# Martinsos/edlib

Hardware: AMD Instinct MI355X
Metric: GCUPS (cell updates/s), 1M x 150bp HW reads vs 5Mb target (higher is better)
Workload: dtype u32

## Files before the change

edlib_amd/csrc/engine.hpp:

```cpp
#pragma once
#include "../../include/edlib_amd.h"
#include "common.hpp"
#include "pair_kernels.hpp"
#include "lanepair.hpp"
#include "reads_kernels.hpp"
#include "cross_kernels.hpp"
#include "window_kernels.hpp"
#include "strands.hpp"

#include <chrono>
#include <deque>
#include <functional>
#include <memory>
#include <vector>

namespace edlib_amd {

struct Tables {
    uint8_t tlut[256];
    uint8_t idToByte[256];
    int sigmaT = 0;
    uint32_t presence[8];
    uint16_t eqtbl[256];
    std::vector<uint8_t> eq8;
// ... 147 lines not shown
    Event evRun0_, evRun1_, evA_, evB_;

    DevBuf<uint8_t> d_in_;
    PinBuf h_in_;
    DevBuf<uint8_t> d_qpool_, d_tpool_, d_tlut_, d_idToByte_, d_eq8_;
    DevBuf<uint16_t> d_eqtbl_;
    hipError_t uploadEq8();
    DevBuf<uint32_t> d_presence_;
    DevBuf<long long> d_qoff_, d_toff_;

    std::vector<int> emptyUnits_, readUnits_, pairUnits_;
    std::vector<int> longUnits_;
    std::vector<int> pairNow_;
    int beginRun(hipError_t guardStatus);
    int enqueueWordSteps();
    int endRun();
    void resetRecords(std::vector<UnitResult>& res);
    void answerEmptyUnits(std::vector<UnitResult>& res);
    int runFlatPhase(std::vector<UnitResult>& res, Lap& lap);
    int runLongReads(std::vector<UnitResult>& res, Lap& lap);
    int runPairPhase(std::vector<UnitResult>& res, Lap& lap);
    int runStartsPhase(std::vector<UnitResult>& res, Lap& lap);
    int runPathsPhase(std::vector<UnitResult>& res, Lap& lap);
    void startStats();
    bool flatDone_ = false;

    struct ReadGroup {
        int nwords = 0, nslots = 0, numSegments = 1, segLen = 0, warm = 0, mMin = 0, mMax = 0;
        std::vector<int> perm;
        DevBuf<int> d_perm, d_qlen, d_kinit, d_alphaExtra, d_segBest, d_segCnt, d_segPos;
        DevBuf<int> d_best, d_total, d_pos, d_flags;
        DevBuf<uint32_t> d_peq;
        bool zeroCopy = false; PinBuf hostOut;
        std::vector<int> ovfSlots; std::vector<long long> ovfOff; DevBuf<int> d_ovfPool;
        DevBuf<int> d_lvMap, d_lvBest, d_lvCnt, d_lvPos; std::vector<int> lvMap; int lvS = 0, lvCap = 0; bool lvValid = false;
        DevBuf<int> d_list;
        int nreal = -1;
        bool mates = false; DevBuf<int> d_win;
    };
    static constexpr int kLastLevelCap = 16;
    int listOpenSlots(ReadGroup& g, int kDone, std::vector<int>& out);
    DevBuf<uint8_t> d_selTmp_;
    std::vector<std::unique_ptr<ReadGroup>> groups_;
    DevBuf<uint32_t> d_tpk_, d_trows_;
    DevBuf<unsigned long long> d_wordSteps_;
    PinBuf h_wordSteps_; bool wordStepsPending_ = false;
    DevBuf<unsigned long long> d_ringSteps_; PinBuf h_ringSteps_; bool ringStepsUsed_ = false;
    unsigned long long* ringStepsCounter();
    bool banded_ = false;
    int syms_ = 4;
    int packTarget();
    int runReads();
    int makeGroup(const std::vector<int>& units, int words, std::unique_ptr<ReadGroup>& g, long long oneRoundWaves = 0);
    int runGroupScans(ReadGroup& g, bool fullOnly);
    int runGroupExact(ReadGroup& g);
    int collectGroup(ReadGroup& g, std::vector<UnitResult>& res);
    int seedThreshold(const ReadGroup& g, bool fullOnly) const;
    int buildSeedIndex();
    int runSeedPass(ReadGroup& g, int k);
    DevBuf<uint32_t> d_seedCnt_, d_seedOff_, d_seedPos_;
    DevBuf<uint8_t> d_seedTmp_;
    bool hits_ = false, hitsHaveRun_ = false;
    HitListBuffers hitList_;
    HitRows hostHits_;
    DevBuf<int> d_hitSlotUnit_;
    DevBuf<long long> d_hitTotal_;
    int runReadHits();
    int scanGroupHits(ReadGroup& g, int slotBase);
    int hitsScanBanded(ReadGroup& g, int slotBase, const int* d_slotmap, int nlanes, int numSegments, int segLen, int warm);
    struct Piece { long long off; int len; int thr; };
    int scanPieces(const std::vector<Piece>& pieces, bool filter, std::vector<std::pair<int, int>>* cand,
                   std::vector<uint8_t>* overflow, std::vector<int>* best);
    int solveLongReads(std::vector<UnitResult>& res, std::vector<int>& fallback);
    bool filterScan_ = false;
    struct ChainArgs { const uint32_t* in = nullptr; uint32_t* out = nullptr; const int* src = nullptr; int inLanes = 0, blocks = 0; const int* rowBase = nullptr; };
    ChainArgs chain_;
    int solveTallFull(const std::vector<int>& units, std::vector<UnitResult>& res, std::vector<int>& handBack);
    int collectReads(std::vector<UnitResult>& res);
    bool readsCollected_ = true;
    int scanGroup(ReadGroup& g, int mode, const int* d_slotmap, int nlanes, int kcap, const int* d_kinit,
                  int numSegments, int segLen, int warm, int* segBest, int* segCnt, int* segPos, int cap,
                  const long long* posOff, const int* posCap, bool unbanded = false,
                  unsigned long long* wordSteps = nullptr, const uint32_t* peqDense = nullptr,
                  const int* qlenDense = nullptr, int peqBottom = 0);

    DevBuf<PairDesc> d_descs_;
    DevBuf<unsigned long long> d_peq64_;
    DevBuf<StoreEntry> d_store_;
    DevBuf<int> d_aux_, d_out3_, d_outScore_, d_outCount_, d_outLast_, d_posPool_, d_opsLen_, d_alpha_;
    DevBuf<uint8_t> d_ops_;
    DevBuf<long long> d_opsOff_;
    int solve(int mode, bool wantPositions, bool wantPath, const std::vector<UnitSpec>& units, SolveOut& out,
              int ring = 0, int ringH = 1);
    int solveChunk(int mode, bool wantPositions, bool wantPath, const std::vector<UnitSpec>& units,
                   size_t a, size_t b, SolveOut& out, int ring, int ringH);
    static const int kWide = -1;
    static const int kRing32 = -2;
    bool ring32_fits(const std::vector<UnitSpec>& units, size_t a, size_t b, int G) const;
    DevBuf<unsigned long long> d_wide_; DevBuf<unsigned> d_wabort_; PinBuf h_wabort_;
    int wideCap_ = -1;
    struct WidePlan { int slots = 1; size_t perLaunch = 1; };
    int planWide(int mode, PairDesc* descs, size_t n, WidePlan& plan);
    int launchWide(int mode, const PairScanArgs& a, const PairDesc* hostDescs, size_t n, const WidePlan& plan);
    int checkWide();
    bool wideSerial_ = false;
    bool wideGateHeld_ = false;
    void wideGateRelease();
    int solveWideSplit(const std::vector<UnitSpec>& units, std::vector<int>& out, int ring = 0);
    struct KnownSplit { long long qoff; int m; long long toff; int T; int score; int row, left, right; };
    std::vector<KnownSplit> knownSplits_;
    int solveGlobalDistances(const std::vector<UnitSpec>& units, std::vector<int>& score, std::vector<OpsOut>* paths = nullptr);
    int solveSemiGlobal(int mode, bool wantPositions, const std::vector<UnitSpec>& units, SolveOut& out);
    int solveSemiGlobalUnits(int mode, bool wantPositions, const std::vector<UnitSpec>& units, SolveOut& out);
    int solveBanded(const BandLadder& ladder, bool wantPositions, const std::vector<UnitSpec>& units, SolveOut& out);
    int alphabetLengthsBegin(hipEvent_t after = nullptr);
    bool alphaDeferred_ = false;
    int alphabetLengthsEnd(std::vector<UnitResult>& res);
    std::vector<int> alphaUnits_; bool alphaOnHost_ = false, alphaPending_ = false; long long alphaBytes_ = 0;
    hipStream_t side_ = nullptr;
    DevBuf<int> d_alphaIdx_, d_alphaOut_; PinBuf alphaPin_;
    struct PathPiece { long long qoff; int m; long long toff; int T; int score; };
    int hirschbergLevel(const std::vector<PathPiece>& big, std::vector<int>& splitRow,
                        std::vector<int>& leftScore, std::vector<int>& rightScore);
    int solvePaths(const std::vector<PathPiece>& jobs, std::vector<OpsOut>& opsOut, std::vector<int>& status);
    std::vector<std::shared_ptr<PinBuf>> opsKeep_;
    std::deque<std::vector<uint8_t>> opsOwned_;

    int qlen(int u) const { return (int)(qoff_[u + 1] - qoff_[u]); }
    long long tbase(int u) const { return shared_ ? toff_[0] : toff_[u]; }
    int tlen(int u) const { return shared_ ? (int)(toff_[1] - toff_[0]) : (int)(toff_[u + 1] - toff_[u]); }

    void scanTimerStart();
    void scanTimerStop();
    std::vector<std::pair<hipEvent_t, hipEvent_t>> scanEvents_;
    size_t scanEventsUsed_ = 0;

    std::vector<UnitResult> results_, work_;
    std::vector<UnitSpec> startUnits_; std::vector<std::pair<int, int>> startWhere_; std::vector<int> live_;
    bool haveResults_ = false;
    long long algoBase_ = -1;
    bool algoDirty_ = false;
    std::vector<int> pairSpecsFor_;
    std::vector<UnitSpec> pairSpecs_, selScratch_; std::vector<size_t> whoScratch_; std::vector<int> lvlScratch_, scoreMain_;
    SolveOut soMain_, soLevel_;
    int pairSpecsVersion_ = 0, levelSpecsVersion_ = -1, shapeVersion_ = -1, alphaIsPairsVersion_ = -1;
    bool alphaIsPairs_ = false;
    struct PairShape { size_t minBlocks = 0, maxBlocks = 0; int minLenLo = 0, minLenHi = 0, maxDiff = 0; } shape_;
    long long levelPeqWords_ = 0;
    bool levelAllReady_ = false;
    PinBuf h_levelSpecs_, h_levelScore_;
    DevBuf<LevelSpec> d_levelSpecs_;
    DevBuf<PairDesc> d_descsAll_;
    DevBuf<unsigned long long> d_peqAll_;
    hipStream_t aux_ = nullptr;
    Event evLevelIn_, evLevelPeq_;
    int prepareLevelAll(const std::vector<UnitSpec>& units);
    std::function<void()> whileScanning_;
    int runLevelAll(const std::vector<UnitSpec>& units, int ring, int ringH, int ringBlocks, int cap, int kcap, int nbMax);
    int laneSpecsVersion_ = -1;
    long long lanePlaneWords_ = -1, laneTgtWords_ = 0;
    bool laneReady_ = false;
    PinBuf h_laneUnits_, h_laneScore_;
    DevBuf<lanepair::LaneUnit> d_laneUnits_;
    DevBuf<lanepair::Plane2> d_lanePlanes_;
    DevBuf<lanepair::Tgt2> d_laneTgts_;
    DevBuf<int> d_laneFlags_, d_laneScore_;
    Event evLanePack_;
// ... 89 lines not shown
```

edlib_amd/csrc/engine_reads.hip:

```cpp
#include "engine.hpp"

#include <algorithm>
#include <chrono>
#include <cmath>
#include <condition_variable>
#include <cstring>
#include <mutex>
#include <thread>

namespace edlib_amd {

__global__ void __launch_bounds__(256)
seed_thresholds_kernel(int* __restrict__ kinit, const int* __restrict__ best, const int* __restrict__ cnt, int n)
{
    const int i = blockIdx.x * blockDim.x + threadIdx.x;
    if (i < n && cnt[i] > 0 && best[i] < kinit[i]) kinit[i] = best[i];
}


int Batch::scanGroup(ReadGroup& g, int mode, const int* d_slotmap, int nlanes, int kcap, const int* d_kinit,
                     int numSegments, int segLen, int warm, int* segBest, int* segCnt, int* segPos, int cap,
                     const long long* posOff, const int* posCap, bool unbanded, unsigned long long* wordSteps,
                     const uint32_t* peqDense, const int* qlenDense, int peqBottom)
{
    ReadScanArgs a{};
    a.peq = peqDense ? peqDense : g.d_peq.p; a.tpk = d_tpk_.p; a.trows = d_trows_.p; a.targetLength = tlen(0);
    if (mode == EDLIB_MODE_SHW) a.targetLength = (int)std::min<long long>(a.targetLength, 64LL * g.nwords + 1);
    a.qlen = qlenDense ? qlenDense : g.d_qlen.p; a.kinit = d_kinit; a.slotmap = d_slotmap; a.nlanes = nlanes;
    a.numSegments = numSegments; a.segLen = segLen; a.warm = warm;
    a.segBest = segBest; a.segCnt = segCnt; a.segPos = segPos; a.cap = cap;
    a.posOff = posOff; a.posCap = posCap;
    a.kcap = kcap; a.wordSteps = wordSteps ? wordSteps : d_wordSteps_.p;
    a.filter = filterScan_ ? 1 : 0;
    a.bottomAligned = peqBottom;
    a.chainIn = chain_.in; a.chainOut = chain_.out; a.chainSrc = chain_.src; a.chainInLanes = chain_.inLanes;
    a.chainBlocks = chain_.blocks; a.rowBase = chain_.rowBase;
    const bool chained = chain_.in != nullptr || chain_.out != nullptr;
    static const bool dbg = getenv("EDLIB_AMD_DEBUG") != nullptr;
    if (dbg) {
        EDLIB_AMD_HIP(hipStreamSynchronize(stream_));
        fprintf(stderr, "[edlib_amd] scanGroup nwords=%d mode=%d nlanes=%d S=%d segLen=%d warm=%d cap=%d kcap=%d slotmap=%p posOff=%p rows=%s\n",
                g.nwords, mode, nlanes, numSegments, segLen, warm, cap, kcap, (const void*)d_slotmap, (const void*)posOff,
                peqBottom > 1 ? "delay" : (peqBottom ? "bottom" : "top"));
    }
    scanTimerStart();
    const bool longGroup = g.nwords > kMaxReadWords;
    const long long colsScanned = std::min<long long>(a.targetLength, (long long)numSegments * segLen) + (long long)(numSegments - 1) * warm;
    const bool fullHeight = banded_ && mode == EDLIB_MODE_HW && unbanded && (chained || syms_ > 4 || longGroup);
    const bool bandedKernel = !fullHeight && banded_ && mode == EDLIB_MODE_HW && (!unbanded || syms_ > 4 || longGroup);
    if (peqBottom && (fullHeight || bandedKernel)) EDLIB_AMD_HIP(hipErrorInvalidValue);
    if (fullHeight) {
        EDLIB_AMD_HIP(launch_scan_reads_full(g.nwords, syms_, a, stream_));
        stats.word_steps += (long long)((nlanes + 63) / 64 * 64) * g.nwords * colsScanned;
    } else if (bandedKernel) EDLIB_AMD_HIP(launch_scan_reads_banded(g.nwords, syms_, a, stream_));
    else {
        EDLIB_AMD_HIP(launch_scan_reads(g.nwords, mode, a, stream_));
        stats.word_steps += (long long)((nlanes + 63) / 64 * 64) * g.nwords * colsScanned;
    }
    scanTimerStop();
    if (dbg) {
        EDLIB_AMD_HIP(hipStreamSynchronize(stream_));
        fprintf(stderr, "[edlib_amd] scanGroup done\n");
    }
    return 0;
}

void plan_segments(int nlanes, int T, int mode, int warmFull, long long wantWaves,
                          int& S, int& segLen, int& warm, int minSegCols)
{
    S = 1; segLen = roundup(T, 16); warm = 0;
    if (mode != EDLIB_MODE_HW) return;
    const long long nrblk = ((long long)nlanes + 63) / 64;
    long long want = (wantWaves + nrblk - 1) / nrblk;
    want = std::max(1LL, std::min<long long>(want, std::min(65535, std::max(1, T / minSegCols))));
    if (warmFull > 0) want = std::max(1LL, std::min<long long>(want, std::max<long long>(1, T / (4LL * warmFull))));
    segLen = roundup((int)((T + want - 1) / want), 16);
    S = (T + segLen - 1) / segLen;
    warm = warmFull;
}

int Batch::runReads()
{
    if (groups_.empty()) return 0;
    stats.path |= 1;
    bool seed = false;
    for (auto& gp : groups_) seed = seed || seedThreshold(*gp, false) >= 0;
    if (seed && buildSeedIndex()) return 1;
    for (auto& gp : groups_) if (runGroupScans(*gp, false)) return 1;
    const int mode = (cfg_.mode == EDLIB_MODE_HW || cfg_.mode == EDLIB_MODE_SHW) ? (int)cfg_.mode : (int)EDLIB_MODE_NW;
    for (auto& gp : groups_)
        if (gp->mates) EDLIB_AMD_HIP(launch_resolve_strands(gp->d_perm.p, gp->d_best.p, gp->d_total.p, gp->nslots, mode, cfg_.k,
                                                            gp->d_win.p, stream_));
    for (auto& gp : groups_) if (runGroupExact(*gp)) return 1;
    return 0;
}

int Batch::runGroupScans(ReadGroup& g, bool fullOnly)
{
    const int T = tlen(0);
    const int mode = (cfg_.mode == EDLIB_MODE_HW || cfg_.mode == EDLIB_MODE_SHW) ? (int)cfg_.mode : (int)EDLIB_MODE_NW;
    const bool banded = banded_ && mode == EDLIB_MODE_HW;
    const int kNoCap = 0x3fffffff;
    static const bool dbgLadder = getenv("EDLIB_AMD_DEBUG") != nullptr;
    EDLIB_AMD_HIP(launch_build_peq_reads(g.nwords, syms_, d_qpool_.p, d_qoff_.p, g.d_perm.p, g.nslots,
                                         d_eqtbl_.p, d_presence_.p, cfg_.k, g.d_peq.p, g.d_qlen.p,
                                         g.d_kinit.p, g.d_alphaExtra.p, stream_));
    const int kSeed = seedThreshold(g, fullOnly);
    const int kFirstMax = kSeed >= 0 ? kSeed : std::max(8, g.nwords / 2);
    int kFirst = (kSeed >= 0 && cfg_.k >= 0) ? std::min(kSeed, cfg_.k) : kFirstMax;
    bool twoPass = !fullOnly && banded && (cfg_.k < 0 || cfg_.k > kFirst) && 32 * g.nwords > kFirst;
    std::vector<int> ladder;
    g.lvValid = false;
    auto probe_scan = [&](const std::vector<int>& map, int kc, std::vector<int>& bestOut) -> int {
        const int nm = (int)map.size();
        int S2, segLen2, warm2;
        plan_segments(nm, T, mode, g.warm, 16384, S2, segLen2, warm2);
// ... 77 lines not shown
        if (runSeedPass(g, kFirst)) return 1;
        if (twoPass) {
            if (listOpenSlots(g, kFirst, todo)) return 1;
            haveTodo = true;
            if (g.nreal < 0) { g.nreal = 0; for (int u : g.perm) g.nreal += u >= 0; }
            if (g.nslots >= 16384 && todo.size() * 10 > (size_t)g.nreal && todo.size() >= 32) {
                const size_t nsm = std::min<size_t>(2048, todo.size());
                std::vector<int> sample(nsm);
                for (size_t i = 0; i < nsm; ++i) sample[i] = todo[i * todo.size() / nsm];
                if (price_ladder(sample, todo.size(), g.nreal)) return 1;
            }
        }
    } else {
        if (scanGroup(g, mode, nullptr, g.nslots, twoPass ? kFirst : kNoCap, g.d_kinit.p, g.numSegments, g.segLen,
                      g.warm, g.d_segBest.p, g.d_segCnt.p, g.d_segPos.p, 8, nullptr, nullptr, fullOnly)) return 1;
        const bool chained = chain_.in != nullptr || chain_.out != nullptr;
        EDLIB_AMD_HIP(launch_merge_segments(g.d_segBest.p, g.d_segCnt.p, g.d_segPos.p, g.numSegments, 8,
                                            g.nslots, nullptr, 16, g.d_best.p, g.d_total.p, g.d_pos.p,
                                            g.d_flags.p, stream_, chained ? kOvfRescan : kOvfGatherGroup));
    }
    ladder.push_back(kNoCap);
    int kDone = kFirst;
    for (size_t lv = 0; twoPass && lv < ladder.size(); ++lv) {
        const int kcapL = ladder[lv];
        const bool last = kcapL == kNoCap;
        if (!haveTodo && listOpenSlots(g, kDone, todo)) return 1;
        haveTodo = false;
        if (todo.empty()) break;
        {
            const size_t no = todo.size();
            int S2, segLen2, warm2;
            plan_segments((int)no, T, mode, g.warm, 65536, S2, segLen2, warm2);
            const size_t items = no * (size_t)S2;
            const int capL = last ? kLastLevelCap : 8;
            EDLIB_AMD_HIP(g.d_lvMap.ensure(no)); EDLIB_AMD_HIP(g.d_lvBest.ensure(items)); EDLIB_AMD_HIP(g.d_lvCnt.ensure(items));
            EDLIB_AMD_HIP(g.d_lvPos.ensure(items * capL));
            int *d_map = g.d_lvMap.p, *d_sb = g.d_lvBest.p, *d_sc = g.d_lvCnt.p, *d_sp = g.d_lvPos.p;
            EDLIB_AMD_HIP(hipMemcpyAsync(d_map, todo.data(), no * sizeof(int), hipMemcpyHostToDevice, stream_));
            bool plain = false;
            if (last && no >= 4096) {
                const int np2 = 64;
                std::vector<int> sub(np2);
                for (int i = 0; i < np2; ++i) sub[i] = todo[(size_t)((long long)i * no / np2)];
                int S3, segLen3, warm3;
                plan_segments(np2, T, mode, g.warm, 16384, S3, segLen3, warm3);
                const size_t it3 = (size_t)np2 * S3;
                DevBuf<int> d_m3, d_b3, d_c3, d_p3; DevBuf<unsigned long long> d_ws;
                EDLIB_AMD_HIP(d_m3.alloc(np2)); EDLIB_AMD_HIP(d_b3.alloc(it3)); EDLIB_AMD_HIP(d_c3.alloc(it3));
                EDLIB_AMD_HIP(d_p3.alloc(it3 * 8)); EDLIB_AMD_HIP(d_ws.alloc(1));
                EDLIB_AMD_HIP(hipMemcpyAsync(d_m3.p, sub.data(), np2 * sizeof(int), hipMemcpyHostToDevice, stream_));
                EDLIB_AMD_HIP(hipMemsetAsync(d_ws.p, 0, sizeof(unsigned long long), stream_));
                if (scanGroup(g, mode, d_m3.p, np2, kNoCap, g.d_kinit.p, S3, segLen3, warm3,
                              d_b3.p, d_c3.p, d_p3.p, 8, nullptr, nullptr, false, d_ws.p)) return 1;
                unsigned long long ws = 0;
                EDLIB_AMD_HIP(hipMemcpyAsync(&ws, d_ws.p, sizeof ws, hipMemcpyDeviceToHost, stream_));
                EDLIB_AMD_HIP(hipStreamSynchronize(stream_));
                const double cols = (double)np2 * ((double)T + (double)(S3 - 1) * warm3);
                plain = (double)ws >= 0.85 * g.nwords * cols;
                stats.word_steps += (long long)ws;
            }
            const bool bottomOk = plain && mode == EDLIB_MODE_HW && syms_ == 4 && g.nwords <= kMaxReadWords &&
                                  chain_.in == nullptr && chain_.out == nullptr;
            const int bottom = !bottomOk ? 0 : (delay_rows_fit(g.nwords, g.mMax) ? 1 + kDelayRows : 1);
            const size_t no64 = (no + 63) / 64 * 64;
            std::vector<int> perm2(no64, -1);
            for (size_t i = 0; i < no; ++i) perm2[i] = g.perm[todo[i]];
            DevBuf<int> d_perm2, d_qlen2, d_kinit2, d_extra2; DevBuf<uint32_t> d_peq2;
            EDLIB_AMD_HIP(d_perm2.alloc(no64)); EDLIB_AMD_HIP(d_qlen2.alloc(no64)); EDLIB_AMD_HIP(d_kinit2.alloc(no64));
            EDLIB_AMD_HIP(d_extra2.alloc(no64)); EDLIB_AMD_HIP(d_peq2.alloc(no64 * (size_t)syms_ * g.nwords));
            EDLIB_AMD_HIP(hipMemcpyAsync(d_perm2.p, perm2.data(), no64 * sizeof(int), hipMemcpyHostToDevice, stream_));
            EDLIB_AMD_HIP(launch_build_peq_reads(g.nwords, syms_, d_qpool_.p, d_qoff_.p, d_perm2.p, (int)no64,
                                                 d_eqtbl_.p, d_presence_.p, cfg_.k, d_peq2.p, d_qlen2.p,
                                                 d_kinit2.p, d_extra2.p, stream_, bottom));
            const int seedCols = 4096;
            DevBuf<int> d_b0, d_c0, d_p0;
            if (mode == EDLIB_MODE_HW && last && no >= 4096 && S2 > 1 && T >= 16 * seedCols) {
                EDLIB_AMD_HIP(d_b0.alloc(no)); EDLIB_AMD_HIP(d_c0.alloc(no)); EDLIB_AMD_HIP(d_p0.alloc(no * 8));
                if (scanGroup(g, mode, nullptr, (int)no, kcapL, d_kinit2.p, 1, seedCols, 0,
                              d_b0.p, d_c0.p, d_p0.p, 8, nullptr, nullptr, plain, nullptr, d_peq2.p, d_qlen2.p, bottom)) return 1;
                hipLaunchKernelGGL(seed_thresholds_kernel, dim3((unsigned)((no + 255) / 256)), dim3(256), 0, stream_,
                                   d_kinit2.p, d_b0.p, d_c0.p, (int)no);
                EDLIB_AMD_HIP(hipGetLastError());
            }
            if (scanGroup(g, mode, nullptr, (int)no, kcapL, d_kinit2.p, S2, segLen2, warm2,
                          d_sb, d_sc, d_sp, capL, nullptr, nullptr, plain, nullptr, d_peq2.p, d_qlen2.p, bottom)) return 1;
            EDLIB_AMD_HIP(launch_merge_segments(d_sb, d_sc, d_sp, S2, capL, (int)no, d_map, 16,
                                                g.d_best.p, g.d_total.p, g.d_pos.p, g.d_flags.p, stream_,
                                                last ? kOvfGatherLevel : kOvfRescan));
            EDLIB_AMD_HIP(hipStreamSynchronize(stream_));
            if (last) { g.lvValid = true; g.lvS = S2; g.lvCap = capL; g.lvMap.swap(todo); }
            if (dbgLadder) fprintf(stderr, "[edlib_amd] level kcap=%d: %zu slots rescanned (plain=%d)\n", kcapL, no, (int)plain);
        }
        kDone = kcapL;
    }
    return 0;
}

int Batch::listOpenSlots(ReadGroup& g, int kDone, std::vector<int>& out)
{
    size_t tmp = 0;
    EDLIB_AMD_HIP(select_slots_scratch_bytes(g.nslots, &tmp));
    EDLIB_AMD_HIP(d_selTmp_.ensure(tmp));
    EDLIB_AMD_HIP(g.d_list.ensure((size_t)g.nslots + 1));
    int* count = g.d_list.p + g.nslots;
    EDLIB_AMD_HIP(launch_select_open_slots(g.d_perm.p, g.d_total.p, g.d_qlen.p, cfg_.k, kDone, g.nslots, g.d_list.p, count,
                                           d_selTmp_.p, d_selTmp_.bytes(), stream_, g.mates));
    int n = 0;
    EDLIB_AMD_HIP(hipMemcpyAsync(&n, count, sizeof(int), hipMemcpyDeviceToHost, stream_));
    EDLIB_AMD_HIP(hipStreamSynchronize(stream_));
    out.resize((size_t)n);
    if (n > 0) {
        EDLIB_AMD_HIP(hipMemcpyAsync(out.data(), g.d_list.p, (size_t)n * sizeof(int), hipMemcpyDeviceToHost, stream_));
        EDLIB_AMD_HIP(hipStreamSynchronize(stream_));
    }
    return 0;
}


int Batch::seedThreshold(const ReadGroup& g, bool fullOnly) const
{
    const long long T = tlen(0);
    if (fullOnly || !banded_ || cfg_.mode != EDLIB_MODE_HW || syms_ != 4 || cfg_.additionalEqualitiesLength > 0 ||
        g.nwords > kMaxReadWords || chain_.in != nullptr || chain_.out != nullptr)
        return -1;
    if (T < 64LL * 32 * g.nwords || g.nslots < 1024 || (long long)g.nslots * T < (1LL << 30)) return -1;
    int kf = -1;
    for (int k = 16; k >= 0 && kf < 0; --k) {
        const int L = g.mMin / (k + 1);
        if (L >= kSeedQ && (double)(k + 1) * (double)T <= std::ldexp(1.0, 2 * L) / 8.0) kf = k;
    }
    return (kf >= 0 && kf >= std::min(8, cfg_.k >= 0 ? cfg_.k : 8)) ? kf : -1;
}

int Batch::buildSeedIndex()
{
    const int T = tlen(0);
    EDLIB_AMD_HIP(d_seedCnt_.ensure((size_t)kSeedBuckets + 1));
    EDLIB_AMD_HIP(d_seedOff_.ensure((size_t)kSeedBuckets + 1));
    EDLIB_AMD_HIP(d_seedPos_.ensure((size_t)T));
    size_t tmp = 0;
    EDLIB_AMD_HIP(seed_index_scratch_bytes(&tmp));
    EDLIB_AMD_HIP(d_seedTmp_.ensure(tmp));
    scanTimerStart();
    EDLIB_AMD_HIP(launch_build_seed_index(d_tpk_.p, T, d_seedCnt_.p, d_seedOff_.p, d_seedPos_.p, d_seedTmp_.p,
                                          d_seedTmp_.bytes(), stream_));
    scanTimerStop();
    return 0;
}

int Batch::runSeedPass(ReadGroup& g, int k)
{
    const int T = tlen(0);
    DevBuf<int> d_back;
    EDLIB_AMD_HIP(d_back.alloc((size_t)g.nslots + 1));
    int* backCount = d_back.p + g.nslots;
    EDLIB_AMD_HIP(hipMemsetAsync(backCount, 0, sizeof(int), stream_));
    SeedArgs a{};
    a.peq = g.d_peq.p; a.qlen = g.d_qlen.p; a.perm = g.d_perm.p; a.tpk = d_tpk_.p; a.targetLength = T;
    a.seedOff = d_seedOff_.p; a.seedPos = d_seedPos_.p; a.nslots = g.nslots; a.k = k;
    a.best = g.d_best.p; a.total = g.d_total.p; a.pos = g.d_pos.p; a.flags = g.d_flags.p;
    a.backSlots = d_back.p; a.backCount = backCount; a.wordSteps = d_wordSteps_.p;
    scanTimerStart();
    EDLIB_AMD_HIP(launch_seed_verify(g.nwords, a, stream_));
    scanTimerStop();
    int nb = 0;
    EDLIB_AMD_HIP(hipMemcpyAsync(&nb, backCount, sizeof(int), hipMemcpyDeviceToHost, stream_));
    EDLIB_AMD_HIP(hipStreamSynchronize(stream_));
    static const bool dbg = getenv("EDLIB_AMD_DEBUG") != nullptr;
// ... 320 lines not shown
```

edlib_amd/csrc/reads_kernels.hip:

```cpp
#include "reads_kernels.hpp"
#include "reads_scan.hpp"
#include "reads_column_asm.hpp"

namespace edlib_amd {


__global__ void __launch_bounds__(256)
pack_target_2bit_kernel(const uint8_t* __restrict__ raw, const uint8_t* __restrict__ lut,
                        int T, u32* __restrict__ tpk, int nwords)
{
    __shared__ uint8_t s_lut[256];
    s_lut[threadIdx.x] = lut[threadIdx.x];
    __syncthreads();
    const int w = blockIdx.x * blockDim.x + threadIdx.x;
    if (w >= nwords) return;
    const int base = w * 16;
    u32 out = 0;
    if (base + 16 <= T) {
        const uint4 v = *reinterpret_cast<const uint4*>(raw + base);
        const u32 d[4] = {v.x, v.y, v.z, v.w};
#pragma unroll
        for (int i = 0; i < 16; ++i)
            out |= (u32)(s_lut[(d[i >> 2] >> ((i & 3) * 8)) & 0xFF] & 3) << (2 * i);
    } else {
// ... 138 lines not shown
    if (syms != 4 && syms != 8 && syms != 16) return hipErrorInvalidValue;
    switch (nwords) {
#define CASE(N) case N: return launch_build_peq_t<N>(reads, qoff, perm, nslots, syms, eqtbl, tpres, kcfg, peq, qlen, kinit, alphaExtra, stream, bottomAlign);
        CASE(1) CASE(2) CASE(3) CASE(4) CASE(5) CASE(6) CASE(7) CASE(8) CASE(10) CASE(12) CASE(14) CASE(16) CASE(24) CASE(32)
#undef CASE
    }
    return hipErrorInvalidValue;
}


#define EDLIB_AMD_DISPATCH_COLUMN(sym)                                                     \
    switch (sym) {                                                                         \
        case 0:  column_step<NWD, MODE, BOTTOM>(E0, Pv, Mv, score, sh, zr0, zr1); asm volatile("; sym0"); break; \
        case 1:  column_step<NWD, MODE, BOTTOM>(E1, Pv, Mv, score, sh, zr0, zr1); asm volatile("; sym1"); break; \
        case 2:  column_step<NWD, MODE, BOTTOM>(E2, Pv, Mv, score, sh, zr0, zr1); asm volatile("; sym2"); break; \
        default: column_step<NWD, MODE, BOTTOM>(E3, Pv, Mv, score, sh, zr0, zr1); asm volatile("; sym3"); break; \
    }

#define EDLIB_AMD_DISPATCH_COLUMN_DELAY(FORM, sym)                                         \
    switch (sym) {                                                                         \
        case 0:  column_step_delay<NWD, FORM>(E0, Pv, Mv, score, nph, nmh, zr0, zr1); asm volatile("; sym0"); break; \
        case 1:  column_step_delay<NWD, FORM>(E1, Pv, Mv, score, nph, nmh, zr0, zr1); asm volatile("; sym1"); break; \
        case 2:  column_step_delay<NWD, FORM>(E2, Pv, Mv, score, nph, nmh, zr0, zr1); asm volatile("; sym2"); break; \
        default: column_step_delay<NWD, FORM>(E3, Pv, Mv, score, nph, nmh, zr0, zr1); asm volatile("; sym3"); break; \
    }

#define EDLIB_AMD_TRACK_SCORE(sc, col)                         \
    if ((sc) <= best) {                                        \
        if ((sc) < best) { best = (sc); cnt = 0; }             \
        if (cnt < cap) pos[cnt] = (col);                       \
        ++cnt;                                                 \
    }
#define EDLIB_AMD_TRACK(col) EDLIB_AMD_TRACK_SCORE(score, col)

template <int NWD, int MODE, bool BOTTOM = false, bool DELAY = false>
__global__ void __launch_bounds__(256)
scan_reads_kernel(const ReadScanArgs a)
{
    static_assert(!DELAY || (BOTTOM && MODE == 2), "delay rows: bottom-aligned HW rows");
    constexpr int kHitGroup = 4;
    static_assert(!DELAY || kHitGroup == kDelayRows + 1, "one nibble per group");
    const int lane = threadIdx.x & 63;
    const int rblk = blockIdx.x * 4 + (threadIdx.x >> 6);
    const int seg = blockIdx.y;
    const int idx = rblk * 64 + lane;
    if (rblk * 64 >= a.nlanes) return;
    const bool live = idx < a.nlanes;
    const int slot = live ? (a.slotmap ? a.slotmap[idx] : idx) : 0;

    u32 E0[NWD], E1[NWD], E2[NWD], E3[NWD], Pv[NWD], Mv[NWD];
    {
        const size_t pb = (size_t)(slot >> 6) * 4 * NWD * 64 + (slot & 63);
#pragma unroll
        for (int d = 0; d < NWD; ++d) {
            E0[d] = a.peq[pb + (size_t)(0 * NWD + d) * 64];
            E1[d] = a.peq[pb + (size_t)(1 * NWD + d) * 64];
            E2[d] = a.peq[pb + (size_t)(2 * NWD + d) * 64];
            E3[d] = a.peq[pb + (size_t)(3 * NWD + d) * 64];
            Pv[d] = ~0u;
            Mv[d] = 0u;
        }
    }
    const int m = a.qlen[slot];
    if constexpr (BOTTOM) {
        const int pad = 32 * NWD - (DELAY ? kDelayRows : 0) - m;
#pragma unroll
        for (int d = 0; d < NWD; ++d) {
            const int lo = pad - 32 * d;
            Pv[d] = lo <= 0 ? ~0u : (lo >= 32 ? 0u : ~0u << lo);
        }
    }
    const u32 sh = (u32)(m - 1) & 31u;
    u32 zr0 = 0, zr1 = 0;
    if constexpr (BOTTOM && (NWD == 4 || NWD == 5)) {
        asm volatile("v_mov_b32 %0, 0" : "=v"(zr0));
        asm volatile("v_mov_b32 %0, 0" : "=v"(zr1));
    }
    int score = m;
    int best = a.kinit[slot];
    int cnt = 0;
    const long long item = (long long)idx * a.numSegments + seg;
    const int cap = !live ? 0 : (a.posCap ? a.posCap[item] : a.cap);
    int* pos = a.segPos + (!live ? 0 : (a.posOff ? a.posOff[item] : item * a.cap));

    const int T = a.targetLength;
    const int c0 = seg * a.segLen;
    int c1 = c0 + a.segLen; if (c1 > T) c1 = T;
    int cw = c0 - a.warm; if (cw < 0) cw = 0;
    cw &= ~15;

    u32 nph = 0, nmh = 0;
    for (int w = cw >> 4; w < (c0 >> 4); ++w) {
        const u32 tw = a.tpk[w];
#pragma unroll
        for (int j = 0; j < 16; ++j) {
            const u32 sym = (tw >> (2 * j)) & 3u;
            if constexpr (!DELAY) {
                EDLIB_AMD_DISPATCH_COLUMN(sym)
            } else if ((j & (kHitGroup - 1)) != kHitGroup - 1) {
                EDLIB_AMD_DISPATCH_COLUMN_DELAY(0, sym)
            } else {
                EDLIB_AMD_DISPATCH_COLUMN_DELAY(1, sym)
            }
        }
    }
    const int wend = c1 >> 4;
    int lim = best + (kHitGroup - 1);
    if constexpr (DELAY) {
        int lim2 = 2 * best + kHitGroup;
        for (int w = c0 >> 4; w < wend; ++w) {
            const u32 tw = a.tpk[w];
#pragma unroll
            for (int j = 0; j < 16; j += kHitGroup) {
#pragma unroll
                for (int q = 0; q < kHitGroup - 1; ++q) {
                    const u32 sym = (tw >> (2 * (j + q))) & 3u;
                    EDLIB_AMD_DISPATCH_COLUMN_DELAY(0, sym)
                }
                const int before = score;
                {
                    const u32 sym = (tw >> (2 * (j + kHitGroup - 1))) & 3u;
                    EDLIB_AMD_DISPATCH_COLUMN_DELAY(1, sym)
                }
                if (__builtin_expect(score + before <= lim2, 0)) {
                    int sc[kHitGroup], acc = before, least = 0x7fffffff;
#pragma unroll
                    for (int q = 0; q < kHitGroup; ++q) {
                        acc += (int)((nph >> (kHitGroup - 1 - q)) & 1u) - (int)((nmh >> (kHitGroup - 1 - q)) & 1u);
                        sc[q] = acc;
                        least = acc < least ? acc : least;
                    }
                    best = (lim2 - kHitGroup) >> 1;
                    if (least <= best) {
#pragma unroll
                        for (int q = 0; q < kHitGroup; ++q) { EDLIB_AMD_TRACK_SCORE(sc[q], w * 16 + j + q) }
                        lim2 = 2 * best + kHitGroup;
                    }
                }
            }
        }
        lim = ((lim2 - kHitGroup) >> 1) + (kHitGroup - 1);
    }
    for (int w = c0 >> 4; !DELAY && w < wend; ++w) {
        const u32 tw = a.tpk[w];
#pragma unroll
        for (int j = 0; j < 16; j += kHitGroup) {
            int sc[kHitGroup];
#pragma unroll
            for (int q = 0; q < kHitGroup; ++q) {
                const u32 sym = (tw >> (2 * (j + q))) & 3u;
                EDLIB_AMD_DISPATCH_COLUMN(sym)
                sc[q] = score;
            }
            if (MODE != 0) {
                if (__builtin_expect(score <= lim, 0)) {
                    best = lim - (kHitGroup - 1);
#pragma unroll
                    for (int q = 0; q < kHitGroup; ++q) { EDLIB_AMD_TRACK_SCORE(sc[q], w * 16 + j + q) }
                    lim = best + (kHitGroup - 1);
                }
            }
        }
    }
    best = lim - (kHitGroup - 1);
    const int rem = c1 - (wend << 4);
    if (rem > 0) {
        u32 tw = a.tpk[wend];
        for (int j = 0; j < rem; ++j) {
            const u32 sym = tw & 3u;
            tw >>= 2;
            if constexpr (DELAY) { EDLIB_AMD_DISPATCH_COLUMN_DELAY(2, sym) } else { EDLIB_AMD_DISPATCH_COLUMN(sym) }
            if (MODE != 0) { EDLIB_AMD_TRACK(wend * 16 + j) }
        }
    }
    if (live) {
        const size_t o = (size_t)idx * a.numSegments + seg;
        a.segBest[o] = (MODE == 0) ? score : best;
        a.segCnt[o] = (MODE == 0) ? 1 : cnt;
    }
}

template <int NWD>
static hipError_t launch_scan_mode(int mode, const ReadScanArgs& a, hipStream_t stream)
{
    const int nrblk = (a.nlanes + 63) / 64;
    dim3 grid((nrblk + 3) / 4, a.numSegments), block(256);
    switch (mode) {
        case 0: hipLaunchKernelGGL((scan_reads_kernel<NWD, 0>), grid, block, 0, stream, a); break;
        case 1: hipLaunchKernelGGL((scan_reads_kernel<NWD, 1>), grid, block, 0, stream, a); break;
        case 2: if (a.bottomAligned == 1 + kDelayRows) hipLaunchKernelGGL((scan_reads_kernel<NWD, 2, true, true>), grid, block, 0, stream, a);
                else if (a.bottomAligned) hipLaunchKernelGGL((scan_reads_kernel<NWD, 2, true>), grid, block, 0, stream, a);
                else hipLaunchKernelGGL((scan_reads_kernel<NWD, 2>), grid, block, 0, stream, a);
                break;
        default: return hipErrorInvalidValue;
    }
    return hipGetLastError();
}

hipError_t launch_scan_reads(int nwords, int mode, const ReadScanArgs& a, hipStream_t stream)
{
    if (a.nlanes == 0) return hipSuccess;
    if (a.bottomAligned && mode != 2) return hipErrorInvalidValue;
    if (a.bottomAligned != 0 && a.bottomAligned != 1 && a.bottomAligned != 1 + kDelayRows) return hipErrorInvalidValue;
    switch (nwords) {
#define CASE(N) case N: return launch_scan_mode<N>(mode, a, stream);
        CASE(1) CASE(2) CASE(3) CASE(4) CASE(5) CASE(6) CASE(7) CASE(8)
#undef CASE
    }
    return hipErrorInvalidValue;
}


hipError_t launch_scan_reads_full_long(int nwords, int syms, const ReadScanArgs& a, hipStream_t stream);
hipError_t launch_scan_reads_banded_long(int nwords, int syms, const ReadScanArgs& a, hipStream_t stream);

template <int S, bool CHAIN>
static hipError_t launch_scan_reads_full_s(int nwords, const ReadScanArgs& a, hipStream_t stream)
{
    dim3 grid((a.nlanes + 63) / 64, a.numSegments), block(64);
    switch (nwords) {
#define CASE(N) case N: EDLIB_AMD_CHECK_STATIC_LDS((scan_reads_full_kernel<N, S, CHAIN>), N * S * 256); \
                        hipLaunchKernelGGL((scan_reads_full_kernel<N, S, CHAIN>), grid, block, 0, stream, a); break;
        CASE(1) CASE(2) CASE(3) CASE(4) CASE(5) CASE(6) CASE(7) CASE(8)
#undef CASE
        default: return hipErrorInvalidValue;
    }
    return hipGetLastError();
}

hipError_t launch_scan_reads_full(int nwords, int syms, const ReadScanArgs& a, hipStream_t stream)
{
    if (a.nlanes == 0) return hipSuccess;
    if (nwords > kMaxReadWords) return launch_scan_reads_full_long(nwords, syms, a, stream);
    const bool chain = a.chainIn != nullptr || a.chainOut != nullptr;
    switch (syms) {
        case 4: return chain ? launch_scan_reads_full_s<4, true>(nwords, a, stream) : launch_scan_reads_full_s<4, false>(nwords, a, stream);
        case 8: return chain ? launch_scan_reads_full_s<8, true>(nwords, a, stream) : launch_scan_reads_full_s<8, false>(nwords, a, stream);
        case 16: return chain ? launch_scan_reads_full_s<16, true>(nwords, a, stream) : launch_scan_reads_full_s<16, false>(nwords, a, stream);
    }
    return hipErrorInvalidValue;
}

template <int S>
static hipError_t launch_scan_reads_banded_s(int nwords, const ReadScanArgs& a, hipStream_t stream)
{
    const int nrblk = (a.nlanes + 63) / 64;
    dim3 grid(nrblk, a.numSegments), block(64);
    switch (nwords) {
#define CASE(N) case N: if (a.filter) { EDLIB_AMD_CHECK_STATIC_LDS((scan_reads_banded_kernel<N, S, true>), N * S * 256); \
                                            hipLaunchKernelGGL((scan_reads_banded_kernel<N, S, true>), grid, block, 0, stream, a); } \
                        else { EDLIB_AMD_CHECK_STATIC_LDS((scan_reads_banded_kernel<N, S, false>), N * S * 256); \
                               hipLaunchKernelGGL((scan_reads_banded_kernel<N, S, false>), grid, block, 0, stream, a); } break;
        CASE(1) CASE(2) CASE(3) CASE(4) CASE(5) CASE(6) CASE(7) CASE(8)
#undef CASE
        default: return hipErrorInvalidValue;
    }
    return hipGetLastError();
}

// ... 163 lines not shown
```

edlib_amd/csrc/reads_kernels.hpp:

```cpp
#pragma once
#include <hip/hip_runtime.h>
#include <stdint.h>

#include "hit_list.hpp"

namespace edlib_amd {

constexpr int kMaxReadWords = 8;
constexpr int kMaxLongReadWords = 16;
constexpr int kMaxLongReadWords4 = 32;
constexpr int kFilterFromWords = 13;
inline int read_group_words(int m) { const int w = (m + 31) / 32; return w <= kMaxReadWords ? w : (w <= 10 ? 10 : (w <= 12 ? 12 : (w <= 14 ? 14 : (w <= 16 ? 16 : (w <= 24 ? 24 : 32))))); }
constexpr int kDelayRows = 3;
constexpr bool delay_rows_fit(int nwords, int longest) { return nwords <= kMaxReadWords && longest >= 1 && longest + kDelayRows <= 32 * nwords; }
constexpr int kLanes = 64;


struct ReadScanArgs {
    const uint32_t* peq;
    const uint32_t* tpk;
    const uint32_t* trows;
    int targetLength;
    const int* qlen;
    const int* kinit;
    const int* slotmap;
    int nlanes;
    int numSegments;
    int segLen;
    int warm;
    int* segBest;
    int* segCnt;
    int* segPos;
    int cap;
    const long long* posOff;
    const int* posCap;
    int kcap;
    unsigned long long* wordSteps;
    const uint32_t* chainIn; uint32_t* chainOut;
    const int* chainSrc;
    int chainInLanes;
    int chainBlocks;
    const int* rowBase;
    int filter;
    HitList hits;
    int slotBase;
    int bottomAligned;
};

hipError_t launch_scan_reads(int nwords, int mode, const ReadScanArgs& a, hipStream_t stream);

hipError_t launch_scan_reads_banded(int nwords, int syms, const ReadScanArgs& a, hipStream_t stream);

hipError_t launch_scan_reads_full(int nwords, int syms, const ReadScanArgs& a, hipStream_t stream);

hipError_t launch_pack_target_2bit(const uint8_t* raw, const uint8_t* lut, int targetLength,
                                   uint32_t* tpk, hipStream_t stream);
hipError_t launch_pack_target_rows(const uint8_t* raw, const uint8_t* lut, int targetLength,
                                   uint32_t* trows, int ndwords, hipStream_t stream);

hipError_t launch_build_peq_reads(int nwords, int syms, const uint8_t* reads, const long long* qoff,
                                  const int* perm, int nslots, const uint16_t* eqtbl,
                                  const uint32_t* targetPresence , int kcfg,
                                  uint32_t* peq, int* qlen, int* kinit, int* alphaExtra,
                                  hipStream_t stream, int bottomAlign = 0);

hipError_t launch_collect_candidates(const int* segCnt, const int* segPos, int numSegments, int cap, int nlanes,
                                     int* out, int maxOut, int* counter, int* overflow, hipStream_t stream);

constexpr int kSeedQ = 12;
constexpr int kSeedBuckets = 1 << (2 * kSeedQ);
constexpr int kSeedBucketCap = 64;
constexpr int kSeedMaxDiag = 32;
constexpr int kSeedMaxWindow = 1024;

struct SeedArgs {
    const uint32_t* peq;
    const int* qlen;
    const int* perm;
    const uint32_t* tpk;
    int targetLength;
    const uint32_t* seedOff;
    const uint32_t* seedPos;
    int nslots;
    int k;
    int* best; int* total; int* pos; int* flags;
    int* backSlots; int* backCount;
    unsigned long long* wordSteps;
    HitList hits;
    int slotBase;
};

hipError_t seed_index_scratch_bytes(size_t* bytes);
hipError_t launch_build_seed_index(const uint32_t* tpk, int targetLength, uint32_t* cnt, uint32_t* off, uint32_t* pos,
                                   void* tmp, size_t tmpBytes, hipStream_t stream);
hipError_t launch_seed_verify(int nwords, const SeedArgs& a, hipStream_t stream);

hipError_t launch_merge_segments(const int* segBest, const int* segCnt, const int* segPos,
                                 int numSegments, int cap, int nlanes, const int* slotmap, int capFinal,
                                 int* best, int* total, int* pos, int* flags, hipStream_t stream, int gatherFlag = 1);
constexpr int kOvfRescan = 1, kOvfGatherLevel = 2, kOvfGatherGroup = 4;
hipError_t launch_gather_segments(const int* segBest, const int* segCnt, const int* segPos, int numSegments, int cap, int n,
                                  const int* idx, const long long* off, const int* lim, int* out, hipStream_t stream);

hipError_t select_slots_scratch_bytes(int nslots, size_t* bytes);
hipError_t launch_select_open_slots(const int* perm, const int* total, const int* qlen, int kcfg, int kDone, int nslots,
                                    int* out, int* count, void* tmp, size_t tmpBytes, hipStream_t stream, bool mates = false);
hipError_t launch_select_flagged_slots(const int* perm, const int* flags, int nslots, int* out, int* count,
                                       void* tmp, size_t tmpBytes, hipStream_t stream, const int* win = nullptr);
hipError_t launch_pick_slot_records(const int* slots, int n, const int* flags, const int* total, int* out, hipStream_t stream);

hipError_t launch_scan_reads_hits(int nwords, int syms, const ReadScanArgs& a, hipStream_t stream);
hipError_t launch_seed_verify_hits(int nwords, const SeedArgs& a, hipStream_t stream);
constexpr int kReadHitsExtraBytes = 12;
hipError_t launch_read_hits_finish(HitListBuffers& hl, const int* slotUnit, int numUnits, long long* total, hipStream_t stream);

}
```

Measured before the change: 3.256 million.

## Share live best score across segments to tighten per-read thresholds during scan

Adds a per-read device buffer that holds the current best edit distance, shared by all segment threads scanning the same read in the bottom-aligned path. Every 1024 columns each thread atomically reads the shared best and tightens its own limit, and it publishes improvements with atomicMin. The aim is to cut wasted hit tracking and candidate recording in segments whose local best is worse than the global one. The cost is extra atomics and periodic loads in the inner scan loop, plus an allocation and device copy per group.

```diff
diff --git a/edlib_amd/csrc/engine.hpp b/edlib_amd/csrc/engine.hpp
--- a/edlib_amd/csrc/engine.hpp
+++ b/edlib_amd/csrc/engine.hpp
@@ -253,7 +253,7 @@
                   int numSegments, int segLen, int warm, int* segBest, int* segCnt, int* segPos, int cap,
                   const long long* posOff, const int* posCap, bool unbanded = false,
                   unsigned long long* wordSteps = nullptr, const uint32_t* peqDense = nullptr,
-                  const int* qlenDense = nullptr, int peqBottom = 0);
+                  const int* qlenDense = nullptr, int peqBottom = 0, int* liveBest = nullptr);
 
     DevBuf<PairDesc> d_descs_;
     DevBuf<unsigned long long> d_peq64_;
diff --git a/edlib_amd/csrc/engine_reads.hip b/edlib_amd/csrc/engine_reads.hip
--- a/edlib_amd/csrc/engine_reads.hip
+++ b/edlib_amd/csrc/engine_reads.hip
@@ -21,7 +21,7 @@
 int Batch::scanGroup(ReadGroup& g, int mode, const int* d_slotmap, int nlanes, int kcap, const int* d_kinit,
                      int numSegments, int segLen, int warm, int* segBest, int* segCnt, int* segPos, int cap,
                      const long long* posOff, const int* posCap, bool unbanded, unsigned long long* wordSteps,
-                     const uint32_t* peqDense, const int* qlenDense, int peqBottom)
+                     const uint32_t* peqDense, const int* qlenDense, int peqBottom, int* liveBest)
 {
     ReadScanArgs a{};
     a.peq = peqDense ? peqDense : g.d_peq.p; a.tpk = d_tpk_.p; a.trows = d_trows_.p; a.targetLength = tlen(0);
@@ -32,6 +32,7 @@
     a.posOff = posOff; a.posCap = posCap;
     a.kcap = kcap; a.wordSteps = wordSteps ? wordSteps : d_wordSteps_.p;
     a.filter = filterScan_ ? 1 : 0;
+    a.liveBest = liveBest;
     a.bottomAligned = peqBottom;
     a.chainIn = chain_.in; a.chainOut = chain_.out; a.chainSrc = chain_.src; a.chainInLanes = chain_.inLanes;
     a.chainBlocks = chain_.blocks; a.rowBase = chain_.rowBase;
@@ -275,8 +276,13 @@
                                    d_kinit2.p, d_b0.p, d_c0.p, (int)no);
                 EDLIB_AMD_HIP(hipGetLastError());
             }
+            DevBuf<int> d_live2;
+            if (bottom && S2 > 1) {
+                EDLIB_AMD_HIP(d_live2.alloc(no64));
+                EDLIB_AMD_HIP(hipMemcpyAsync(d_live2.p, d_kinit2.p, no64 * sizeof(int), hipMemcpyDeviceToDevice, stream_));
+            }
             if (scanGroup(g, mode, nullptr, (int)no, kcapL, d_kinit2.p, S2, segLen2, warm2,
-                          d_sb, d_sc, d_sp, capL, nullptr, nullptr, plain, nullptr, d_peq2.p, d_qlen2.p, bottom)) return 1;
+                          d_sb, d_sc, d_sp, capL, nullptr, nullptr, plain, nullptr, d_peq2.p, d_qlen2.p, bottom, d_live2.p)) return 1;
             EDLIB_AMD_HIP(launch_merge_segments(d_sb, d_sc, d_sp, S2, capL, (int)no, d_map, 16,
                                                 g.d_best.p, g.d_total.p, g.d_pos.p, g.d_flags.p, stream_,
                                                 last ? kOvfGatherLevel : kOvfRescan));
diff --git a/edlib_amd/csrc/reads_kernels.hip b/edlib_amd/csrc/reads_kernels.hip
--- a/edlib_amd/csrc/reads_kernels.hip
+++ b/edlib_amd/csrc/reads_kernels.hip
@@ -244,6 +244,12 @@
     const long long item = (long long)idx * a.numSegments + seg;
     const int cap = !live ? 0 : (a.posCap ? a.posCap[item] : a.cap);
     int* pos = a.segPos + (!live ? 0 : (a.posOff ? a.posOff[item] : item * a.cap));
+    constexpr int kLiveBlocks = kLivePeriod / 16;
+    constexpr int kNoImport = 0x1fffffff;
+    int* const livep = BOTTOM ? a.liveBest : nullptr;
+    int lidx = idx;
+    if constexpr (BOTTOM) asm volatile("" : "+v"(lidx));
+#define EDLIB_AMD_LIVE_LOAD() (live ? __hip_atomic_load(livep + lidx, __ATOMIC_RELAXED, __HIP_MEMORY_SCOPE_AGENT) : kNoImport)
 
     const int T = a.targetLength;
     const int c0 = seg * a.segLen;
@@ -270,7 +276,13 @@
     int lim = best + (kHitGroup - 1);
     if constexpr (DELAY) {
         int lim2 = 2 * best + kHitGroup;
-        for (int w = c0 >> 4; w < wend; ++w) {
+        for (int w0 = c0 >> 4; w0 < wend; w0 += kLiveBlocks) {
+        if (livep) {
+            const int got = EDLIB_AMD_LIVE_LOAD();
+            if (2 * got + kHitGroup < lim2) { lim2 = 2 * got + kHitGroup; cnt = 0; }
+        }
+        const int w1 = w0 + kLiveBlocks < wend ? w0 + kLiveBlocks : wend;
+        for (int w = w0; w < w1; ++w) {
             const u32 tw = a.tpk[w];
 #pragma unroll
             for (int j = 0; j < 16; j += kHitGroup) {
@@ -296,14 +308,22 @@
                     if (least <= best) {
 #pragma unroll
                         for (int q = 0; q < kHitGroup; ++q) { EDLIB_AMD_TRACK_SCORE(sc[q], w * 16 + j + q) }
+                        if (livep && live && 2 * best + kHitGroup < lim2) atomicMin(livep + lidx, best);
                         lim2 = 2 * best + kHitGroup;
                     }
                 }
             }
         }
+        }
         lim = ((lim2 - kHitGroup) >> 1) + (kHitGroup - 1);
     }
-    for (int w = c0 >> 4; !DELAY && w < wend; ++w) {
+    for (int w0 = c0 >> 4; !DELAY && w0 < wend; w0 += kLiveBlocks) {
+    if (livep) {
+        const int got = EDLIB_AMD_LIVE_LOAD();
+        if (got + (kHitGroup - 1) < lim) { lim = got + (kHitGroup - 1); cnt = 0; }
+    }
+    const int w1 = w0 + kLiveBlocks < wend ? w0 + kLiveBlocks : wend;
+    for (int w = w0; w < w1; ++w) {
         const u32 tw = a.tpk[w];
 #pragma unroll
         for (int j = 0; j < 16; j += kHitGroup) {
@@ -319,11 +339,14 @@
                     best = lim - (kHitGroup - 1);
 #pragma unroll
                     for (int q = 0; q < kHitGroup; ++q) { EDLIB_AMD_TRACK_SCORE(sc[q], w * 16 + j + q) }
+                    if (livep && live && best + (kHitGroup - 1) < lim) atomicMin(livep + lidx, best);
                     lim = best + (kHitGroup - 1);
                 }
             }
         }
     }
+    }
+#undef EDLIB_AMD_LIVE_LOAD
     best = lim - (kHitGroup - 1);
     const int rem = c1 - (wend << 4);
     if (rem > 0) {
@@ -336,7 +359,7 @@
         }
     }
     if (live) {
-        const size_t o = (size_t)idx * a.numSegments + seg;
+        const size_t o = (size_t)lidx * a.numSegments + seg;
         a.segBest[o] = (MODE == 0) ? score : best;
         a.segCnt[o] = (MODE == 0) ? 1 : cnt;
     }
diff --git a/edlib_amd/csrc/reads_kernels.hpp b/edlib_amd/csrc/reads_kernels.hpp
--- a/edlib_amd/csrc/reads_kernels.hpp
+++ b/edlib_amd/csrc/reads_kernels.hpp
@@ -45,7 +45,9 @@
     HitList hits;
     int slotBase;
     int bottomAligned;
+    int* liveBest;
 };
+constexpr int kLivePeriod = 1024;
 
 hipError_t launch_scan_reads(int nwords, int mode, const ReadScanArgs& a, hipStream_t stream);
 
```

New measurement: 3.303 million, median of 6. 1.01x the previous value.
